# freiberg-roman/mj-grasp-sim

Measured on AMD Instinct MI355X. Metric: grasp candidates evaluated/sec at 200-step horizon, Robotiq2F85xYCB, higher is better.
Workload: dtype f64

## Files before the change

mj-grasp-sim_amd/csrc/mgs_kernels.hip:

```cpp

#include <hip/hip_runtime.h>
#include <stdint.h>

#include "../../include/mgs_gpu.h"

#define K_MINVAL 1e-15
#define K_MAXF 16
#define K_MAXPOLY 40
#define K_POLY_POINTS (4 * K_MAXF + 3 * K_MAXPOLY)
#define K_MPR_MAXIT 64
#define K_FEAT_EPS 1e-5
#define K_BB_MERGE 1e-6
#define K_CERT 8
#define CERT_W 17
#define CERT_STORE 1e-6
#define CERT_EPS 1e-10
#define WAVE 64
#ifndef MGS_GPAD
#ifdef MGS_G_GLOBAL
#define MGS_GPAD 0
#else
#define MGS_GPAD 1
#endif
#endif
// ... 2423 lines not shown
#pragma unroll
  for (int k = 0; k < 3; k++) { a[k] = c.cx1[k]; b[k] = c.cx2[k]; }
}
template <int HW>
DEVI void support_pairq(const PairCtxQ<HW>& c, const double* dir, double* out1, double* out2) {
  const int lane = lane_id(), side = (lane / HW) & 1, li = lane % HW, hb = lane - li;
  double sd[3] = {side ? -dir[0] : dir[0], side ? -dir[1] : dir[1], side ? -dir[2] : dir[2]};
  double dl[3];
  mulmtv3(dl, c.R, sd);
  SupAcc a;
  sup_init(a);
  if (li < c.n) {
    double sc = (c.c[0] * dl[0] + c.c[1] * dl[1]) + c.c[2] * dl[2];
    if (sc > a.best) { a.best = sc; a.bi = li; a.vx = c.c[0]; a.vy = c.c[1]; a.vz = c.c[2]; }
  }
  const int P = c.P;
  double m = a.best;
  if (P > 1) m = max_f64(m, dpp_d(m, 0));
  if (P > 2) m = max_f64(m, dpp_d(m, 1));
  if (P > 4) m = max_f64(m, dpp_d(m, 2));
  if (HW > 8 && P > 8) m = max_f64(m, dpp_d(m, 3));
  const double M = shfl(m, hb);
  const unsigned long long tied = __ballot(a.bi != 0x7fffffff && a.best == M);
  const unsigned tr = (unsigned)(tied >> hb) & ((1u << HW) - 1u);
  const int src = hb + (tr ? __ffs(tr) - 1 : 0);
  double v[3] = {shfl(a.vx, src), shfl(a.vy, src), shfl(a.vz, src)};
  double t[3], wv[3];
  mulmv3(t, c.R, v);
  add3(wv, c.x, t);
  if (c.r > 0.0) { wv[0] = wv[0] + c.r * sd[0]; wv[1] = wv[1] + c.r * sd[1]; wv[2] = wv[2] + c.r * sd[2]; }
  const int s1 = lane - (lane % (2 * HW)), s2 = s1 + HW;
#pragma unroll
  for (int k = 0; k < 3; k++) {
    out1[k] = shfl(wv[k], s1);
    out2[k] = shfl(wv[k], s2);
  }
}
template <int HW>
DEVI void mink_support(const PairCtxQ<HW>& c, const double* dir, SupPt* p, unsigned long long) {
  PT(4);
  PCNT(28, 1);
  support_pairq<HW>(c, dir, p->a, p->b);
  sub3(p->v, p->a, p->b);
  PT(22);
}
#define MQ_P1 0
#define MQ_P2 1
#define MQ_DISC 2
#define MQ_REF 3
#define MQ_PEN 4
#define MQ_FIN 5
#define MQ_DONE 6
template <class QC>
DEVI int ccd_mpr_q(const Mdl& md, const Dat& d, const QC& pc, double* n, double* depth, double* pos) {
  const double tol = md.m.mpr_tolerance;
  const int maxit = md.m.ccd_iterations;
  SupPt p0, p1, p2, p3, ps;
  double dir[3];
  int ph = MQ_P1, it = 0, hit = 0;
  mpr_centres(pc, d, 0, 0, p0.a, p0.b);
  sub3(p0.v, p0.a, p0.b);
  if (ccd_vzero(p0.v)) p0.v[0] = p0.v[0] + CCD_EPS * 10.0;
  dir[0] = -p0.v[0]; dir[1] = -p0.v[1]; dir[2] = -p0.v[2];
  ccd_normalize(dir);
  p1 = p0; p2 = p0; p3 = p0;
  for (;;) {
    if (ph == MQ_REF || ph == MQ_PEN) {
      ccd_portal_dir(dir, p1, p2, p3);
      if (ph == MQ_REF) {
        const double dt = dot3(dir, p1.v);
        if (ccd_iszero(dt) || dt > 0.0) { ph = MQ_PEN; it = 0; }
      }
    }
    const unsigned long long act = __ballot(ph < MQ_FIN);
    if (!act) break;
    mink_support(pc, dir, &ps, act);
    const double dt = dot3(ps.v, dir);
    if (ph == MQ_P1) {
      if (ccd_iszero(dt) || dt < 0.0) {
        ph = MQ_DONE;
      } else {
        p1 = ps;
        cross3(dir, p0.v, p1.v);
        if (ccd_iszero(dot3(dir, dir))) {
          if (!ccd_vzero(p1.v)) {
#pragma unroll
            for (int k = 0; k < 3; k++) { n[k] = p1.v[k]; pos[k] = (p1.a[k] + p1.b[k]) * 0.5; }
            *depth = sqrt(dot3(n, n));
            ccd_normalize(n);
            hit = 1;
          }
          ph = MQ_DONE;
        } else {
          ccd_normalize(dir);
          ph = MQ_P2;
        }
      }
    } else if (ph == MQ_P2) {
      if (ccd_iszero(dt) || dt < 0.0) {
        ph = MQ_DONE;
      } else {
        p2 = ps;
        double e1[3], e2[3];
        sub3(e1, p1.v, p0.v);
        sub3(e2, p2.v, p0.v);
        cross3(dir, e1, e2);
        ccd_normalize(dir);
        if (dot3(dir, p0.v) > 0.0) {
          SupPt tmp = p1; p1 = p2; p2 = tmp;
          dir[0] = -dir[0]; dir[1] = -dir[1]; dir[2] = -dir[2];
        }
        ph = MQ_DISC;
        it = 0;
      }
    } else if (ph == MQ_DISC) {
      if (ccd_iszero(dt) || dt < 0.0) {
        ph = MQ_DONE;
      } else {
        p3 = ps;
        double c[3];
        int cont = 0;
        cross3(c, p1.v, p3.v);
        double dc = dot3(c, p0.v);
        if (dc < 0.0 && !ccd_iszero(dc)) { p2 = p3; cont = 1; }
        if (!cont) {
          cross3(c, p3.v, p2.v);
          dc = dot3(c, p0.v);
          if (dc < 0.0 && !ccd_iszero(dc)) { p1 = p3; cont = 1; }
        }
        if (!cont) {
          ph = MQ_REF;
          it = 0;
        } else {
          double e1[3], e2[3];
          sub3(e1, p1.v, p0.v);
          sub3(e2, p2.v, p0.v);
          cross3(dir, e1, e2);
          ccd_normalize(dir);
          if (++it == CCD_MAXLOOP) ph = MQ_DONE;
        }
      }
    } else if (ph == MQ_REF) {
      if (!(ccd_iszero(dt) || dt > 0.0) || ccd_reach_tol(p1, p2, p3, ps, dir, tol)) {
        ph = MQ_DONE;
      } else {
        PORTAL_EXPAND(p0, p1, p2, p3, ps);
        if (++it == CCD_MAXLOOP) ph = MQ_DONE;
      }
    } else if (ph == MQ_PEN) {
      if (ccd_reach_tol(p1, p2, p3, ps, dir, tol) || it > maxit) {
        ph = MQ_FIN;
      } else {
        PORTAL_EXPAND(p0, p1, p2, p3, ps);
        it++;
      }
    }
  }
  double w[3], fp[3];
  const double dep = sqrt(ccd_tri_dist2(p1.v, p2.v, p3.v, w));
  ccd_normalize(w);
  ccd_find_pos(p0, p1, p2, p3, fp);
  if (ph == MQ_FIN && !ccd_iszero(dep)) {
#pragma unroll
    for (int k = 0; k < 3; k++) { n[k] = w[k]; pos[k] = fp[k]; }
    *depth = dep;
    hit = 1;
  }
  return hit;
}

#define MCCD_N 40
#define MCCD_RES 48
#define MCCD_RES2 96
DEVI void mccd_store(Dat& d, int at, int hit, const double* n, const double* pos, const double* cd, double depth,
                     double cm) {
  double* o = (double*)d.poly + at;
#pragma unroll
  for (int i = 0; i < 3; i++) { o[i] = n[i]; o[3 + i] = pos[i]; o[6 + i] = cd[i]; }
  o[9] = depth;
  o[10] = cm;
  o[11] = hit ? 1.0 : 0.0;
}
DEVI void mccd_take_groups(const Mdl& md, Dat& d, int pair, int g1, int g2, int ngroups, int& nc) {
  const double* cp = (const double*)d.poly;
  const int ncmax = md.m.ncon_max;
#pragma unroll 1
  for (int k = 0; k < ngroups; k++) {
    const double* r = cp + MCCD_RES + 12 * k;
    if (r[11] == 0.0) continue;
    double pk[3] = {r[3], r[4], r[5]};
    if (!mccd_is_new(d, nc, pk, mccd_tol(md, g1, g2))) continue;
    double nk[3] = {r[0], r[1], r[2]};
    const double dk = r[9];
    mccd_list_add(d, nc, pk);
    nc++;
    double u1[3], u2[3];
    make_frame(nk, u1, u2);
    if (lane_id() == 0) add_contact(d, ncmax, pair, g1, g2, pk, nk, u1, u2, -dk);
  }
  wsync();
}
template <int HW>
DEVI void multiccd_q(const Mdl& md, Dat& d, int pair, int g1, int g2, const double* n, const double* pos) {
  constexpr int G = WAVE / (2 * HW);
  mccd_list_init(d, pos);
  int nc = 1;
#pragma unroll 1
  for (int q0 = 0; q0 < 4; q0 += G) {
    {
      double t1[3], t2[3];
      make_frame(n, t1, t2);
      PairCtxQ<HW> pc;
      pair_ctxq<HW>(md, d, g1, g2, t1, t2, pos, q0, pc);
      double nn[3], dd = 0.0, pp[3], dir[3] = {0.0, 0.0, 0.0}, cmx = -1.0;
      const int hit = ccd_mpr_q(md, d, pc, nn, &dd, pp);
      const int lane = lane_id();
      if (lane % (2 * HW) == 0) mccd_store(d, MCCD_RES + 12 * (lane / (2 * HW)), hit, nn, pp, dir, dd, cmx);
      wsync();
    }
    mccd_take_groups(md, d, pair, g1, g2, G, nc);
  }
  wsync();
}

#define MCCD_POSE 16
DEVI void mccd_perturb(const Dat& d, Dat& dw, int g1, int g2, const double* n, const double* pv, int q, int at) {
  const int ax = q >> 1, sg = q & 1;
  double t1[3], t2[3];
  make_frame(n, t1, t2);
  double axis[3] = {ax ? t2[0] : t1[0], ax ? t2[1] : t1[1], ax ? t2[2] : t1[2]};
  double s = sg ? MCCD_S : -MCCD_S;
  double* out = (double*)dw.poly + at;
#pragma unroll 1
  for (int side = 0; side < 2; side++) {
    const int g = side ? g2 : g1;
    double qq[4];
    qq[0] = MCCD_C;
    if (side) { qq[1] = -(axis[0] * s); qq[2] = -(axis[1] * s); qq[3] = -(axis[2] * s); }
    else { qq[1] = axis[0] * s; qq[2] = axis[1] * s; qq[3] = axis[2] * s; }
    double M[9], R[9], xg[3], r[3], t[3], xo[3];
#pragma unroll
    for (int k = 0; k < 9; k++) R[k] = d.geom_xmat[9 * g + k];
#pragma unroll
    for (int k = 0; k < 3; k++) xg[k] = d.geom_xpos[3 * g + k];
    quat2mat(M, qq);
    mulmm3(R, M, R);
    sub3(r, xg, pv);
    mulmv3(t, M, r);
    add3(xo, t, pv);
    if (lane_id() == 0) {
#pragma unroll
      for (int k = 0; k < 9; k++) out[9 * side + k] = R[k];
#pragma unroll
      for (int k = 0; k < 3; k++) out[18 + 3 * side + k] = xo[k];
    }
  }
  wsync();
}

#ifndef MGS_MCCD_W
#define MGS_MCCD_W 1
#endif
#define MCCD_POSEW 128
struct PairCtxW {
  PairCtx base;
  const double* pose;
  double cx1[3], cx2[3];
};
DEVI void mpr_centres(const PairCtxW& c, const Dat&, int, int, double* a, double* b) {
#pragma unroll
  for (int k = 0; k < 3; k++) { a[k] = c.cx1[k]; b[k] = c.cx2[k]; }
}
DEVI void mink_support(const PairCtxW& c, const double* dir, SupPt* p, unsigned long long act) {
  const int grp = lane_id() >> 4;
#pragma unroll 1
  for (int g = 0; g < 4; g++) {
    if (!((act >> (16 * g)) & 1ull)) continue;
    double dg[3] = {readlane_d(dir[0], 16 * g), readlane_d(dir[1], 16 * g), readlane_d(dir[2], 16 * g)};
    PairCtx q = c.base;
    const double* P = c.pose + 24 * g;
#pragma unroll
    for (int k = 0; k < 9; k++) { q.R1[k] = P[k]; q.R2[k] = P[9 + k]; }
#pragma unroll
    for (int k = 0; k < 3; k++) { q.x1[k] = P[18 + k]; q.x2[k] = P[21 + k]; }
    SupPt t;
    mink_support(q, dg, &t);
    if (grp == g) {
#pragma unroll
      for (int k = 0; k < 3; k++) { p->a[k] = t.a[k]; p->b[k] = t.b[k]; }
    }
  }
  sub3(p->v, p->a, p->b);
}
#ifndef MGS_MCCD_G
#define MGS_MCCD_G 1
#endif
#ifndef GS_CH
#define GS_CH 4
#endif
struct PairCtxG {
  int n1, n2;
  int nmax1, nmax2;
  const double *V1, *V2;
  double c1[3], c2[3];
  double r1, r2;
  double cy1[2], cy2[2];
  const double* pose;
  double cx1[3], cx2[3];
};
DEVI void pair_ctxg(const Mdl& md, int g1, int g2, const double* pose, PairCtxG& c) {
  const int li = lane_id() & 15;
  const int32_t *ghull = IA(md, geom_hullid), *hadr = IA(md, hull_vertadr), *hnum = IA(md, hull_vertnum);
  const int h1 = ghull[g1], h2 = ghull[g2];
  c.n1 = hnum[h1];
  c.n2 = hnum[h2];
  c.nmax1 = c.n1;
  c.nmax2 = c.n2;
  c.V1 = DA(md, hull_vert) + 3 * hadr[h1];
  c.V2 = DA(md, hull_vert) + 3 * hadr[h2];
  const int i1 = li < c.n1 ? li : 0, i2 = li < c.n2 ? li : 0;
#pragma unroll
  for (int k = 0; k < 3; k++) { c.c1[k] = c.V1[k * c.n1 + i1]; c.c2[k] = c.V2[k * c.n2 + i2]; }
  c.r1 = DA(md, geom_radius)[g1];
  c.r2 = DA(md, geom_radius)[g2];
  const double* cy = DA(md, geom_cyl);
  c.cy1[0] = cy[2 * g1]; c.cy1[1] = cy[2 * g1 + 1];
  c.cy2[0] = cy[2 * g2]; c.cy2[1] = cy[2 * g2 + 1];
  c.pose = pose;
#pragma unroll
  for (int k = 0; k < 3; k++) { c.cx1[k] = pose[18 + k]; c.cx2[k] = pose[21 + k]; }
}
DEVI void mpr_centres(const PairCtxG& c, const Dat&, int, int, double* a, double* b) {
#pragma unroll
  for (int k = 0; k < 3; k++) { a[k] = c.cx1[k]; b[k] = c.cx2[k]; }
}
DEVI int dpp_i(int x, int ctrl_sel) {
  switch (ctrl_sel) {
    case 0: return __builtin_amdgcn_mov_dpp(x, 0xB1, 0xF, 0xF, false);
    case 1: return __builtin_amdgcn_mov_dpp(x, 0x4E, 0xF, 0xF, false);
    case 2: return __builtin_amdgcn_mov_dpp(x, 0x141, 0xF, 0xF, false);
    default: return __builtin_amdgcn_mov_dpp(x, 0x140, 0xF, 0xF, false);
  }
}
DEVI void sup_group(int n, int nmax, const double* V, const double* cached, const double* dl, double* v) {
  const int lane = lane_id(), li = lane & 15;
  SupAcc a;
  sup_init(a);
  if (nmax <= 16) {
    if (li < n) {
      double sc = (cached[0] * dl[0] + cached[1] * dl[1]) + cached[2] * dl[2];
      if (sc > a.best) { a.best = sc; a.bi = li; a.vx = cached[0]; a.vy = cached[1]; a.vz = cached[2]; }
    }
  } else {
#pragma unroll 1
    for (int base = 0; base < nmax; base += GS_CH * 16) {
      double x[GS_CH], y[GS_CH], z[GS_CH];
#pragma unroll
      for (int u = 0; u < GS_CH; u++) {
        const int i = base + u * 16 + li;
        const int ii = i < n ? i : 0;
        x[u] = V[ii]; y[u] = V[n + ii]; z[u] = V[2 * n + ii];
      }
#pragma unroll
      for (int u = 0; u < GS_CH; u++) {
        const int i = base + u * 16 + li;
        double sc = (x[u] * dl[0] + y[u] * dl[1]) + z[u] * dl[2];
        if (i < n && sc > a.best) { a.best = sc; a.bi = i; a.vx = x[u]; a.vy = y[u]; a.vz = z[u]; }
      }
    }
  }
  double m = a.best;
  m = max_f64(m, dpp_d(m, 0));
  m = max_f64(m, dpp_d(m, 1));
  m = max_f64(m, dpp_d(m, 2));
  m = max_f64(m, dpp_d(m, 3));
  int w = a.best == m ? a.bi : 0x7fffffff, t;
  t = dpp_i(w, 0); w = t < w ? t : w;
  t = dpp_i(w, 1); w = t < w ? t : w;
  t = dpp_i(w, 2); w = t < w ? t : w;
  t = dpp_i(w, 3); w = t < w ? t : w;
  if (w == 0x7fffffff) w = 0;
  const int src = (lane - li) + (w & 15);
  v[0] = shfl(a.vx, src);
  v[1] = shfl(a.vy, src);
  v[2] = shfl(a.vz, src);
}
DEVI void support_pairg(const PairCtxG& c, const double* dir, double* out1, double* out2) {
  const double* P = c.pose;
  double nd[3] = {-dir[0], -dir[1], -dir[2]};
  double R[9], dl[3], v[3], t[3], x[3];
#pragma unroll
  for (int k = 0; k < 9; k++) R[k] = P[k];
  mulmtv3(dl, R, dir);
  sup_group(c.n1, c.nmax1, c.V1, c.c1, dl, v);
  if (c.cy1[0] > 0.0) cyl_support(v, c.cy1, dl);
#pragma unroll
  for (int k = 0; k < 3; k++) x[k] = P[18 + k];
  mulmv3(t, R, v);
  add3(out1, x, t);
  if (c.r1 > 0.0) { out1[0] = out1[0] + c.r1 * dir[0]; out1[1] = out1[1] + c.r1 * dir[1]; out1[2] = out1[2] + c.r1 * dir[2]; }
#pragma unroll
  for (int k = 0; k < 9; k++) R[k] = P[9 + k];
  mulmtv3(dl, R, nd);
  sup_group(c.n2, c.nmax2, c.V2, c.c2, dl, v);
  if (c.cy2[0] > 0.0) cyl_support(v, c.cy2, dl);
#pragma unroll
  for (int k = 0; k < 3; k++) x[k] = P[21 + k];
  mulmv3(t, R, v);
  add3(out2, x, t);
  if (c.r2 > 0.0) { out2[0] = out2[0] + c.r2 * nd[0]; out2[1] = out2[1] + c.r2 * nd[1]; out2[2] = out2[2] + c.r2 * nd[2]; }
}
DEVI void mink_support(const PairCtxG& c, const double* dir, SupPt* p, unsigned long long) {
  PT(4);
  PCNT(28, 1);
  PCNT(29, (c.n1 > WAVE) + (c.n2 > WAVE));
  support_pairg(c, dir, p->a, p->b);
  sub3(p->v, p->a, p->b);
  if (c.n1 > WAVE || c.n2 > WAVE) PT(39); else PT(22);
}
DEVI void multiccd_w(const Mdl& md, Dat& d, int pair, int g1, int g2, const double* n, const double* pos) {
  mccd_list_init(d, pos);
#pragma unroll 1
  for (int q = 0; q < 4; q++) mccd_perturb(d, d, g1, g2, n, pos, q, MCCD_POSEW + 24 * q);
  const int lane = lane_id(), grp = lane >> 4;
  {
#if MGS_MCCD_G
    PairCtxG pc;
    pair_ctxg(md, g1, g2, (const double*)d.poly + MCCD_POSEW + 24 * grp, pc);
#else
    PairCtxW pc;
    pair_ctx(md, d, g1, g2, pc.base);
    pc.pose = (const double*)d.poly + MCCD_POSEW;
    const double* P = pc.pose + 24 * grp;
#pragma unroll
    for (int k = 0; k < 3; k++) { pc.cx1[k] = P[18 + k]; pc.cx2[k] = P[21 + k]; }
#endif
    double nn[3], dd = 0.0, pp[3], dir[3] = {0.0, 0.0, 0.0};
    const int hit = ccd_mpr_q(md, d, pc, nn, &dd, pp);
    if ((lane & 15) == 0) mccd_store(d, MCCD_RES + 12 * grp, hit, nn, pp, dir, dd, -1.0);
    wsync();
  }
  int nc = 1;
  mccd_take_groups(md, d, pair, g1, g2, 4, nc);
}

DEVI void collide_convex_mj(const Mdl& md, Dat& d, int pairA, int pairB, int mccd) {
  const int lane = lane_id();
  const int32_t *p1 = IA(md, pair_geom1), *p2 = IA(md, pair_geom2);
  const int32_t *ghull = IA(md, geom_hullid), *hnum = IA(md, hull_vertnum);
  const double* cy = DA(md, geom_cyl);
  const int ncmax = md.m.ncon_max;
  if (pairB >= 0) {
    const int gA1 = p1[pairA], gA2 = p2[pairA], gB1 = p1[pairB], gB2 = p2[pairB];
    PairCtx2 q;
    pair_ctx2(md, d, gA1, gA2, gB1, gB2, q);
    const int g1 = lane < 32 ? gA1 : gB1, g2 = lane < 32 ? gA2 : gB2;
    double n[3], depth, pos[3], cd[3], cm;
    const int hit = ccd_mpr(md, d, q, g1, g2, n, &depth, pos, cd, &cm);
    if ((lane & 31) == 0) mccd_store(d, MCCD_RES2 + 12 * (lane >> 5), hit, n, pos, cd, depth, cm);
    wsync();
  }
  const int np = pairB >= 0 ? 2 : 1;
  const double* cp = (const double*)d.poly;
#pragma unroll 1
  for (int k = 0; k < np; k++) {
    const int pair = k ? pairB : pairA;
    const int G1 = p1[pair], G2 = p2[pair];
    const bool multi = mccd && md.m.ccd_mode == MGS_CCD_MULTI && IA(md, pair_kind)[pair] == MGS_PAIR_CONVEX;
    int nc = 0;
#pragma unroll 1
    for (int it = 0; it < 5; it++) {
      if (it > 0 || pairB < 0) {
        PairCtx pc;
        if (it > 0) {
          mccd_perturb(d, d, G1, G2, cp + MCCD_N, cp, it - 1, MCCD_POSE);
          const double* pz = cp + MCCD_POSE;
          pair_ctx_pose(md, G1, G2, pz, pz + 18, pz + 9, pz + 21, pc);
        } else {
          pair_ctx(md, d, G1, G2, pc);
        }
        double n[3], depth, pos[3], cd[3], cm;
        const int hit = ccd_mpr(md, d, pc, G1, G2, n, &depth, pos, cd, &cm);
        wsync();
        if (lane == 0) mccd_store(d, MCCD_RES, hit, n, pos, cd, depth, cm);
        wsync();
      }
      const double* r = it == 0 && pairB >= 0 ? cp + MCCD_RES2 + 12 * k : cp + MCCD_RES;
      const int hk = r[11] != 0.0;
      if (it == 0) {
        PT(4);
        cert_update(md, d, pair, G1, G2, hk, r + 6, r[10]);
        PCNT(26, 1);
        PCNT(27, hk);
        if (!hk) break;
        double t1[3], t2[3];
        make_frame(r, t1, t2);
        if (lane == 0) add_contact(d, ncmax, pair, G1, G2, r + 3, r, t1, t2, -r[9]);
        wsync();
        if (!multi) break;
        const int nm1 = hnum[ghull[G1]], nm2 = hnum[ghull[G2]];
        const bool cyl = cy[2 * G1] > 0.0 || cy[2 * G2] > 0.0;
        if (MGS_MCCD_Q && !cyl && nm1 <= 8 && nm2 <= 8) {
          double n0[3] = {r[0], r[1], r[2]}, p0[3] = {r[3], r[4], r[5]};
          multiccd_q<8>(md, d, pair, G1, G2, n0, p0);
          break;
        }
        if (MGS_MCCD_W) {
          double n0[3] = {r[0], r[1], r[2]}, p0[3] = {r[3], r[4], r[5]};
          multiccd_w(md, d, pair, G1, G2, n0, p0);
          break;
        }
        if (lane == 0) {
          double* w = (double*)d.poly;
#pragma unroll
          for (int i = 0; i < 3; i++) { w[i] = r[3 + i]; w[MCCD_N + i] = r[i]; }
        }
        wsync();
        nc = 1;
      } else {
        if (!hk) continue;
        double pk[3] = {r[3], r[4], r[5]};
        if (!mccd_is_new(d, nc, pk, mccd_tol(md, G1, G2))) continue;
        double nk[3] = {r[0], r[1], r[2]};
        const double dk = r[9];
        mccd_list_add(d, nc, pk);
        nc++;
        double u1[3], u2[3];
        make_frame(nk, u1, u2);
        if (lane == 0) add_contact(d, ncmax, pair, G1, G2, pk, nk, u1, u2, -dk);
      }
    }
    wsync();
  }
  PT(41);
}

DEVI double kdist3(const double* a, const double* b) {
  double dx[3];
  sub3(dx, a, b);
  return sqrt(dot3(dx, dx));
}
DEVI int raw_sphere_sphere(const double* p1, const double* z1, double r1, const double* p2, const double* z2,
                           double r2, double margin, double* pos, double* n, double* dist) {
  double dd = (kdist3(p1, p2) - r1) - r2;
  if (dd > margin) return 0;
  sub3(n, p2, p1);
  if (normalize3(n) < K_MINVAL) {
    cross3(n, z1, z2);
    normalize3(n);
  }
  double s = r1 + 0.5 * dd;
#pragma unroll
  for (int k = 0; k < 3; k++) pos[k] = p1[k] + n[k] * s;
  *dist = dd;
// ... 282 lines not shown
  for (int k = 0; k < 3; k++)
#pragma unroll
    for (int i = 0; i < 3; i++) { A1[3 * k + i] = R1[3 * i + k]; A2[3 * k + i] = R2[3 * i + k]; }
  const int qa = q < 6 ? 0 : (q - 6) / 3, qb = q < 6 ? 0 : (q - 6) % 3;
  const double* Rf = q < 3 ? R1 : R2;
  const int kf = q < 3 ? q : (q < 6 ? q - 3 : 0);
  double e1[3], e2[3], L[3], cx[3];
#pragma unroll
  for (int i = 0; i < 3; i++) {
    e1[i] = R1[3 * i + qa];
    e2[i] = R2[3 * i + qb];
  }
  cross3(cx, e1, e2);
#pragma unroll
  for (int i = 0; i < 3; i++) L[i] = q < 6 ? Rf[3 * i + kf] : cx[i];
  double ll = dot3(L, L);
  if (ll < 1e-20) return 0;
  double r1 = (h1[0] * fabs(dot3(A1, L)) + h1[1] * fabs(dot3(A1 + 3, L))) + h1[2] * fabs(dot3(A1 + 6, L));
  double r2 = (h2[0] * fabs(dot3(A2, L)) + h2[1] * fabs(dot3(A2 + 3, L))) + h2[2] * fabs(dot3(A2 + 6, L));
  return fabs(dot3(D, L)) > (r1 + r2) + (margin + 1e-12) * sqrt(ll);
}

DEVI unsigned long long obb_separated_wave(const Dat& d, unsigned long long am, int g1, int g2, const double* D,
                                           const double* h1, const double* h2, double margin) {
  const int lane = lane_id(), grp = lane >> 4, q = lane & 15;
  unsigned long long sep = 0ull;
  while (am) {
    unsigned long long m = am;
    for (int t = 0; t < grp; t++) m &= m - 1ull;
    int b = m ? __ffsll((long long)m) - 1 : 0;
    int G1 = shfl(g1, b), G2 = shfl(g2, b);
    double Db[3], h1b[3], h2b[3];
#pragma unroll
    for (int i = 0; i < 3; i++) {
      Db[i] = shfl(D[i], b);
      h1b[i] = shfl(h1[i], b);
      h2b[i] = shfl(h2[i], b);
    }
    double mb = shfl(margin, b);
    int s = 0;
    if (m && q < 15) s = obb_axis_separated(q, d.geom_xmat + 9 * G1, d.geom_xmat + 9 * G2, Db, h1b, h2b, mb);
    unsigned long long sm = __ballot(s);
#pragma unroll
    for (int k = 0; k < 4; k++) {
      if (!am) break;
      int bk = __ffsll((long long)am) - 1;
      if ((sm >> (16 * k)) & 0x7fffull) sep |= 1ull << bk;
      am &= am - 1ull;
    }
  }
  return sep;
}

DEVI void collision(const Mdl& md, Dat& d, int mccd = 1) {
  int lane = lane_id();
  const int32_t *p1 = IA(md, pair_geom1), *p2 = IA(md, pair_geom2);
  const double *aabb = DA(md, geom_aabb), *pm = DA(md, pair_margin);
  if (lane == 0) d.NCON = 0;
  wsync();
  int npair = md.m.npair;
  for (int c0 = 0; c0 < npair; c0 += WAVE) {
    int p = c0 + lane;
    int ov = 0;
    int g[2] = {0, 0};
    double c[2][3], hw[2][3], D[3] = {0.0, 0.0, 0.0}, h[2][3] = {{0.0, 0.0, 0.0}, {0.0, 0.0, 0.0}}, mp = 0.0;
    if (p < npair) {
      g[0] = p1[p];
      g[1] = p2[p];
      mp = pm[p];
      for (int s = 0; s < 2; s++) {
        const double* R = d.geom_xmat + 9 * g[s];
        const double* lc = aabb + 6 * g[s];
        const double* lh = lc + 3;
        double t[3];
        mulmv3(t, R, lc);
        add3(c[s], d.geom_xpos + 3 * g[s], t);
        for (int k = 0; k < 3; k++) {
          h[s][k] = lh[k];
          hw[s][k] = (fabs(R[3 * k]) * lh[0] + fabs(R[3 * k + 1]) * lh[1]) + fabs(R[3 * k + 2]) * lh[2];
        }
      }
      ov = 1;
      for (int k = 0; k < 3; k++)
        if (fabs(c[0][k] - c[1][k]) > (hw[0][k] + hw[1][k]) + mp) ov = 0;
      sub3(D, c[1], c[0]);
    }
    PT(59);
    int small2 = 0;
    const int pk = p < npair ? IA(md, pair_kind)[p] : MGS_PAIR_BOXBOX;
    const bool mpr_pair = md.m.ccd_mode == MGS_CCD_R5 ? pk != MGS_PAIR_BOXBOX
                                                       : (pk == MGS_PAIR_CONVEX || pk == MGS_PAIR_CONVEX_SMOOTH);
    if (ov && mpr_pair) {
      const int32_t *ghull = IA(md, geom_hullid), *hnum = IA(md, hull_vertnum);
      small2 = hnum[ghull[g[0]]] <= 16 && hnum[ghull[g[1]]] <= 16;
    }
    const unsigned long long smallm = __ballot(small2);
    unsigned long long mask = __ballot(ov);
    mask &= ~obb_separated_wave(d, mask, g[0], g[1], D, h[0], h[1], mp);
    PT(60);
    mask &= ~cert_check(md, d, c0, mask);
    PT(3);
    while (mask) {
      int b = __ffsll((long long)mask) - 1;
      mask &= mask - 1ull;
      const int kind = IA(md, pair_kind)[c0 + b];
      if (((smallm >> b) & 1ull) && mask && ((smallm >> (__ffsll((long long)mask) - 1)) & 1ull)) {
        int b2 = __ffsll((long long)mask) - 1;
        mask &= mask - 1ull;
        if (md.m.ccd_mode == MGS_CCD_R5) collide_pair2(md, d, c0 + b, c0 + b2);
        else collide_convex_mj(md, d, c0 + b, c0 + b2, mccd);
      } else if (kind == MGS_PAIR_BOXBOX) {
        collide_boxbox(md, d, c0 + b);
      } else if (md.m.ccd_mode == MGS_CCD_R5) {
        collide_pair(md, d, c0 + b);
      } else if (kind == MGS_PAIR_CONVEX || kind == MGS_PAIR_CONVEX_SMOOTH) {
        collide_convex_mj(md, d, c0 + b, -1, mccd);
      } else {
        collide_prim(md, d, c0 + b, kind);
      }
    }
  }
}

enum {
  L_qpos, L_qvel, L_qacc_ws, L_ctrl, L_mocap_pos, L_mocap_quat, L_time, L_act, L_act_dot,
  L_xpos, L_xquat, L_xmat, L_subtree_com, L_cinert, L_cdof,
  L_M, L_Dv, L_Dinv, L_sD, L_isD, L_tmp, L_tmp2,
  L_qfrc_smooth, L_qacc_smooth, L_qfrc_constraint,
  L_act_force, L_act_moment, L_act_length, L_act_vel,
  L_con_pos, L_con_frame, L_con_dist, L_con_mu, L_con_blk,
  L_efc_R, L_efc_b, L_cert,
  L_U, L_ints, L_COUNT
};
enum {
  U_poly, U_pdep, U_geom_xpos, U_geom_xmat, U_xipos, U_xanchor, U_xaxis, U_subtree_mass, U_comacc,
  U_crb, U_cvel, U_cacc, U_cfrc, U_cdof_dot, U_qfrc_bias, U_qfrc_passive, U_qfrc_actuator,
  U_G, U_aref, U_vel, U_pos, U_margin, U_nH, U_scratch, U_jar, U_jv, U_f, U_Dr, U_isR, U_nw, U_nw0, U_ng,
  U_ndir, U_qDeriv, U_COUNT
};
#ifndef MGS_HBM_EXTRA
#define MGS_HBM_EXTRA 0
#endif
DEVI size_t hbm_slice(int ne, int nv, int nc) {
  return (size_t)ne * nv + (MGS_HBM_EXTRA ? (size_t)(K_CERT * CERT_W + 9 * nc + BLKSTRIDE * nc) : 0);
}
struct Lay {
  int o[L_COUNT];
  int u[U_COUNT];
  int ncon_max, nefc_max, nv;
  int total_doubles;
  double* gmem;
};

#ifdef MGS_SPECIAL
#include MGS_SPECIAL
static_assert(MGS_SL_ABI == MGS_ABI_VERSION, "specialisation header of another ABI version: regenerate it");
static_assert(MGS_SL_DESC_BYTES == sizeof(mgs_model_desc), "specialisation header of another mgs_model_desc");
#else
#define MGS_SL_NV 0
constexpr int mgs_sl_words[L_COUNT + U_COUNT + 4] = {0};
constexpr mgs_model_desc mgs_sl_desc = {};
#endif
static_assert(sizeof(mgs_sl_words) == sizeof(int) * (L_COUNT + U_COUNT + 4), "specialised layout size");

template <int SL>
DEVI void bind(Dat& d, double* s, const Lay& l) {
#define LO(k) (SL ? mgs_sl_words[k] : l.o[k])
#define LU(k) (SL ? mgs_sl_words[L_COUNT + (k)] : l.u[k])
#define B(f) d.f = s + LO(L_##f)
  B(qpos); B(qvel); B(qacc_ws); B(ctrl); B(mocap_pos); B(mocap_quat); B(time); B(act); B(act_dot);
  B(xpos); B(xquat); B(xmat); B(subtree_com); B(cinert); B(cdof);
// ... 2761 lines not shown
```

Measured before the change: 391,900.

## Batch first MPR of up to four convex pairs across 16-lane groups

Adds collide_chunk_mj, which runs the initial MPR for up to four overlapping convex pairs at once, one pair per 16-lane group, then processes each pair's contact, cert update and multi-CCD perturbation from the stored results. Previously pairs were handled one or two at a time with the whole wave busy on each. ccd_mpr_q now also returns the last direction and a separation certificate value, and skips the final portal distance work when no lane finished in penetration. Per-group radius and cylinder data move from registers into shared scratch. The cost is more scratch-layout coupling and extra wave syncs, and some groups sit idle when fewer than four convex pairs are available.

```diff
diff --git a/mj-grasp-sim_amd/csrc/mgs_kernels.hip b/mj-grasp-sim_amd/csrc/mgs_kernels.hip
--- a/mj-grasp-sim_amd/csrc/mgs_kernels.hip
+++ b/mj-grasp-sim_amd/csrc/mgs_kernels.hip
@@ -2499,12 +2499,13 @@
 #define MQ_FIN 5
 #define MQ_DONE 6
 template <class QC>
-DEVI int ccd_mpr_q(const Mdl& md, const Dat& d, const QC& pc, double* n, double* depth, double* pos) {
+DEVI int ccd_mpr_q(const Mdl& md, const Dat& d, const QC& pc, double* n, double* depth, double* pos, double* cd,
+                   double* cm, int live = 1) {
   const double tol = md.m.mpr_tolerance;
   const int maxit = md.m.ccd_iterations;
   SupPt p0, p1, p2, p3, ps;
-  double dir[3];
-  int ph = MQ_P1, it = 0, hit = 0;
+  double dir[3], cert = -1.0;
+  int ph = live ? MQ_P1 : MQ_DONE, it = 0, hit = 0;
   mpr_centres(pc, d, 0, 0, p0.a, p0.b);
   sub3(p0.v, p0.a, p0.b);
   if (ccd_vzero(p0.v)) p0.v[0] = p0.v[0] + CCD_EPS * 10.0;
@@ -2525,6 +2526,7 @@
     const double dt = dot3(ps.v, dir);
     if (ph == MQ_P1) {
       if (ccd_iszero(dt) || dt < 0.0) {
+        cert = -dt;
         ph = MQ_DONE;
       } else {
         p1 = ps;
@@ -2545,6 +2547,7 @@
       }
     } else if (ph == MQ_P2) {
       if (ccd_iszero(dt) || dt < 0.0) {
+        cert = -dt;
         ph = MQ_DONE;
       } else {
         p2 = ps;
@@ -2562,6 +2565,7 @@
       }
     } else if (ph == MQ_DISC) {
       if (ccd_iszero(dt) || dt < 0.0) {
+        cert = -dt;
         ph = MQ_DONE;
       } else {
         p3 = ps;
@@ -2588,7 +2592,10 @@
         }
       }
     } else if (ph == MQ_REF) {
-      if (!(ccd_iszero(dt) || dt > 0.0) || ccd_reach_tol(p1, p2, p3, ps, dir, tol)) {
+      if (!(ccd_iszero(dt) || dt > 0.0)) {
+        cert = -dt;
+        ph = MQ_DONE;
+      } else if (ccd_reach_tol(p1, p2, p3, ps, dir, tol)) {
         ph = MQ_DONE;
       } else {
         PORTAL_EXPAND(p0, p1, p2, p3, ps);
@@ -2603,16 +2610,20 @@
       }
     }
   }
-  double w[3], fp[3];
-  const double dep = sqrt(ccd_tri_dist2(p1.v, p2.v, p3.v, w));
-  ccd_normalize(w);
-  ccd_find_pos(p0, p1, p2, p3, fp);
-  if (ph == MQ_FIN && !ccd_iszero(dep)) {
-#pragma unroll
-    for (int k = 0; k < 3; k++) { n[k] = w[k]; pos[k] = fp[k]; }
-    *depth = dep;
-    hit = 1;
-  }
+  if (__ballot(ph == MQ_FIN)) {
+    double w[3], fp[3];
+    const double dep = sqrt(ccd_tri_dist2(p1.v, p2.v, p3.v, w));
+    ccd_normalize(w);
+    ccd_find_pos(p0, p1, p2, p3, fp);
+    if (ph == MQ_FIN && !ccd_iszero(dep)) {
+#pragma unroll
+      for (int k = 0; k < 3; k++) { n[k] = w[k]; pos[k] = fp[k]; }
+      *depth = dep;
+      hit = 1;
+    }
+  }
+  cd[0] = dir[0]; cd[1] = dir[1]; cd[2] = dir[2];
+  *cm = cert;
   return hit;
 }
 
@@ -2660,7 +2671,7 @@
       PairCtxQ<HW> pc;
       pair_ctxq<HW>(md, d, g1, g2, t1, t2, pos, q0, pc);
       double nn[3], dd = 0.0, pp[3], dir[3] = {0.0, 0.0, 0.0}, cmx = -1.0;
-      const int hit = ccd_mpr_q(md, d, pc, nn, &dd, pp);
+      const int hit = ccd_mpr_q(md, d, pc, nn, &dd, pp, dir, &cmx);
       const int lane = lane_id();
       if (lane % (2 * HW) == 0) mccd_store(d, MCCD_RES + 12 * (lane / (2 * HW)), hit, nn, pp, dir, dd, cmx);
       wsync();
@@ -2709,6 +2720,7 @@
 #define MGS_MCCD_W 1
 #endif
 #define MCCD_POSEW 128
+#define MCCD_GEO 224
 struct PairCtxW {
   PairCtx base;
   const double* pose;
@@ -2750,12 +2762,11 @@
   int nmax1, nmax2;
   const double *V1, *V2;
   double c1[3], c2[3];
-  double r1, r2;
-  double cy1[2], cy2[2];
+  const double* geo;
   const double* pose;
   double cx1[3], cx2[3];
 };
-DEVI void pair_ctxg(const Mdl& md, int g1, int g2, const double* pose, PairCtxG& c) {
+DEVI void pair_ctxg(const Mdl& md, int g1, int g2, const double* pose, double* geo, PairCtxG& c) {
   const int li = lane_id() & 15;
   const int32_t *ghull = IA(md, geom_hullid), *hadr = IA(md, hull_vertadr), *hnum = IA(md, hull_vertnum);
   const int h1 = ghull[g1], h2 = ghull[g2];
@@ -2768,11 +2779,12 @@
   const int i1 = li < c.n1 ? li : 0, i2 = li < c.n2 ? li : 0;
 #pragma unroll
   for (int k = 0; k < 3; k++) { c.c1[k] = c.V1[k * c.n1 + i1]; c.c2[k] = c.V2[k * c.n2 + i2]; }
-  c.r1 = DA(md, geom_radius)[g1];
-  c.r2 = DA(md, geom_radius)[g2];
-  const double* cy = DA(md, geom_cyl);
-  c.cy1[0] = cy[2 * g1]; c.cy1[1] = cy[2 * g1 + 1];
-  c.cy2[0] = cy[2 * g2]; c.cy2[1] = cy[2 * g2 + 1];
+  if (li < 6) {
+    const int g = (li == 0 || li == 2 || li == 3) ? g1 : g2;
+    geo[li] = li < 2 ? DA(md, geom_radius)[g] : DA(md, geom_cyl)[2 * g + (li & 1)];
+  }
+  wsync();
+  c.geo = geo;
   c.pose = pose;
 #pragma unroll
   for (int k = 0; k < 3; k++) { c.cx1[k] = pose[18 + k]; c.cx2[k] = pose[21 + k]; }
@@ -2840,22 +2852,23 @@
   for (int k = 0; k < 9; k++) R[k] = P[k];
   mulmtv3(dl, R, dir);
   sup_group(c.n1, c.nmax1, c.V1, c.c1, dl, v);
-  if (c.cy1[0] > 0.0) cyl_support(v, c.cy1, dl);
+  if (c.geo[2] > 0.0) cyl_support(v, c.geo + 2, dl);
 #pragma unroll
   for (int k = 0; k < 3; k++) x[k] = P[18 + k];
   mulmv3(t, R, v);
   add3(out1, x, t);
-  if (c.r1 > 0.0) { out1[0] = out1[0] + c.r1 * dir[0]; out1[1] = out1[1] + c.r1 * dir[1]; out1[2] = out1[2] + c.r1 * dir[2]; }
+  const double r1 = c.geo[0], r2 = c.geo[1];
+  if (r1 > 0.0) { out1[0] = out1[0] + r1 * dir[0]; out1[1] = out1[1] + r1 * dir[1]; out1[2] = out1[2] + r1 * dir[2]; }
 #pragma unroll
   for (int k = 0; k < 9; k++) R[k] = P[9 + k];
   mulmtv3(dl, R, nd);
   sup_group(c.n2, c.nmax2, c.V2, c.c2, dl, v);
-  if (c.cy2[0] > 0.0) cyl_support(v, c.cy2, dl);
+  if (c.geo[4] > 0.0) cyl_support(v, c.geo + 4, dl);
 #pragma unroll
   for (int k = 0; k < 3; k++) x[k] = P[21 + k];
   mulmv3(t, R, v);
   add3(out2, x, t);
-  if (c.r2 > 0.0) { out2[0] = out2[0] + c.r2 * nd[0]; out2[1] = out2[1] + c.r2 * nd[1]; out2[2] = out2[2] + c.r2 * nd[2]; }
+  if (r2 > 0.0) { out2[0] = out2[0] + r2 * nd[0]; out2[1] = out2[1] + r2 * nd[1]; out2[2] = out2[2] + r2 * nd[2]; }
 }
 DEVI void mink_support(const PairCtxG& c, const double* dir, SupPt* p, unsigned long long) {
   PT(4);
@@ -2873,7 +2886,7 @@
   {
 #if MGS_MCCD_G
     PairCtxG pc;
-    pair_ctxg(md, g1, g2, (const double*)d.poly + MCCD_POSEW + 24 * grp, pc);
+    pair_ctxg(md, g1, g2, (const double*)d.poly + MCCD_POSEW + 24 * grp, (double*)d.poly + MCCD_GEO + 6 * grp, pc);
 #else
     PairCtxW pc;
     pair_ctx(md, d, g1, g2, pc.base);
@@ -2882,9 +2895,9 @@
 #pragma unroll
     for (int k = 0; k < 3; k++) { pc.cx1[k] = P[18 + k]; pc.cx2[k] = P[21 + k]; }
 #endif
-    double nn[3], dd = 0.0, pp[3], dir[3] = {0.0, 0.0, 0.0};
-    const int hit = ccd_mpr_q(md, d, pc, nn, &dd, pp);
-    if ((lane & 15) == 0) mccd_store(d, MCCD_RES + 12 * grp, hit, nn, pp, dir, dd, -1.0);
+    double nn[3], dd = 0.0, pp[3], dir[3], cmx;
+    const int hit = ccd_mpr_q(md, d, pc, nn, &dd, pp, dir, &cmx);
+    if ((lane & 15) == 0) mccd_store(d, MCCD_RES + 12 * grp, hit, nn, pp, dir, dd, cmx);
     wsync();
   }
   int nc = 1;
@@ -3335,6 +3348,129 @@
   return sep;
 }
 
+#ifndef MGS_MPR1_G
+#ifdef MGS_WAVES_PER_EU
+#define MGS_MPR1_G 0
+#else
+#define MGS_MPR1_G 1
+#endif
+#endif
+#if MGS_MPR1_G && !(MGS_MCCD_W && MGS_MCCD_G)
+#error "MGS_MPR1_G 1 shares multiccd_w's group-scan MPR call site: it needs MGS_MCCD_W 1 and MGS_MCCD_G 1"
+#endif
+#define MPR1_POSE (K_POLY_POINTS * 3 - 4 * 24)
+#define MPR1_RES (MPR1_POSE - 4 * 12)
+static_assert(MPR1_POSE + 4 * 24 == K_POLY_POINTS * 3, "the first-MPR block ends with the polygon scratch");
+static_assert(MPR1_RES >= MCCD_GEO + 4 * 6 && MCCD_GEO >= MCCD_POSEW + 4 * 24 && MPR1_RES >= MCCD_RES + 4 * 12 &&
+                  MCCD_GEO >= 3 * 48,
+              "the first-MPR block overlaps multiccd's or collide_boxbox's scratch");
+#if MGS_MPR1_G
+DEVI void collide_chunk_mj(const Mdl& md, Dat& d, int c0, unsigned long long mask, unsigned long long cvx, int mccd) {
+  const int lane = lane_id(), grp = lane >> 4, li = lane & 15;
+  const int32_t *p1 = IA(md, pair_geom1), *p2 = IA(md, pair_geom2);
+  const int32_t *ghull = IA(md, geom_hullid), *hnum = IA(md, hull_vertnum);
+  const double* cy = DA(md, geom_cyl);
+  const int ncmax = md.m.ncon_max;
+  double* cp = (double*)d.poly;
+  unsigned long long batch = 0ull;
+  while (mask) {
+    const int b = __ffsll((long long)mask) - 1;
+    const int pair = c0 + b;
+    if (!((cvx >> b) & 1ull)) {
+      const int kind = IA(md, pair_kind)[pair];
+      if (kind == MGS_PAIR_BOXBOX) collide_boxbox(md, d, pair);
+      else collide_prim(md, d, pair, kind);
+      mask &= mask - 1ull;
+      continue;
+    }
+    const int G1 = p1[pair], G2 = p2[pair];
+    const bool multi = mccd && md.m.ccd_mode == MGS_CCD_MULTI && IA(md, pair_kind)[pair] == MGS_PAIR_CONVEX;
+#pragma unroll 1
+    for (int st = 0; st < 2; st++) {
+      int ga = G1, gb = G2, live = 1, at = MCCD_RES + 12 * grp, posat = MCCD_POSEW + 24 * grp;
+      if (st == 0) {
+        if ((batch >> b) & 1ull) continue;
+        unsigned long long m = mask & cvx;
+        int bg = -1;
+        batch = 0ull;
+#pragma unroll
+        for (int k = 0; k < 4; k++) {
+          if (!m) break;
+          const int bk = __ffsll((long long)m) - 1;
+          m &= m - 1ull;
+          batch |= 1ull << bk;
+          if (grp == k) bg = bk;
+        }
+        live = bg >= 0;
+        if (!live) bg = b;
+        ga = p1[c0 + bg];
+        gb = p2[c0 + bg];
+        at = MPR1_RES + 12 * grp;
+        posat = MPR1_POSE + 24 * grp;
+#pragma unroll
+        for (int u = 0; u < 2; u++) {
+          const int v = li + 16 * u;
+          if (v < 24) {
+            double x;
+            if (v < 9) x = d.geom_xmat[9 * ga + v];
+            else if (v < 18) x = d.geom_xmat[9 * gb + (v - 9)];
+            else if (v < 21) x = d.geom_xpos[3 * ga + (v - 18)];
+            else x = d.geom_xpos[3 * gb + (v - 21)];
+            cp[posat + v] = x;
+          }
+        }
+        wsync();
+      } else {
+        const double* r = cp + MPR1_RES + 12 * __popcll(batch & ((1ull << b) - 1ull));
+        const int hk = r[11] != 0.0;
+        PT(4);
+        cert_update(md, d, pair, G1, G2, hk, r + 6, r[10]);
+        PCNT(26, 1);
+        PCNT(27, hk);
+        if (!hk) continue;
+        double t1[3], t2[3];
+        make_frame(r, t1, t2);
+        if (lane == 0) add_contact(d, ncmax, pair, G1, G2, r + 3, r, t1, t2, -r[9]);
+        wsync();
+        if (!multi) continue;
+        const int nm1 = hnum[ghull[G1]], nm2 = hnum[ghull[G2]];
+        const bool cyl = cy[2 * G1] > 0.0 || cy[2 * G2] > 0.0;
+        double n0[3] = {r[0], r[1], r[2]}, p0[3] = {r[3], r[4], r[5]};
+        if (MGS_MCCD_Q && !cyl && nm1 <= 8 && nm2 <= 8) {
+          multiccd_q<8>(md, d, pair, G1, G2, n0, p0);
+          continue;
+        }
+        mccd_list_init(d, p0);
+#pragma unroll 1
+        for (int q = 0; q < 4; q++) mccd_perturb(d, d, G1, G2, n0, p0, q, MCCD_POSEW + 24 * q);
+      }
+      {
+        PairCtxG pc;
+        pair_ctxg(md, ga, gb, cp + posat, cp + MCCD_GEO + 6 * grp, pc);
+#pragma unroll
+        for (int k = 1; k < 4; k++) {
+          const int a1 = __builtin_amdgcn_readlane(pc.n1, 16 * k), a2 = __builtin_amdgcn_readlane(pc.n2, 16 * k);
+          pc.nmax1 = a1 > pc.nmax1 ? a1 : pc.nmax1;
+          pc.nmax2 = a2 > pc.nmax2 ? a2 : pc.nmax2;
+        }
+        pc.nmax1 = __builtin_amdgcn_readfirstlane(pc.nmax1);
+        pc.nmax2 = __builtin_amdgcn_readfirstlane(pc.nmax2);
+        double nn[3], dd = 0.0, pp[3], cd[3], cm;
+        const int hit = ccd_mpr_q(md, d, pc, nn, &dd, pp, cd, &cm, live);
+        if (li == 0 && live) mccd_store(d, at, hit, nn, pp, cd, dd, cm);
+        wsync();
+      }
+      if (st == 1) {
+        int nc = 1;
+        mccd_take_groups(md, d, pair, G1, G2, 4, nc);
+      }
+    }
+    PT(41);
+    mask &= mask - 1ull;
+  }
+}
+#endif
+
 DEVI void collision(const Mdl& md, Dat& d, int mccd = 1) {
   int lane = lane_id();
   const int32_t *p1 = IA(md, pair_geom1), *p2 = IA(md, pair_geom2);
@@ -3373,7 +3509,7 @@
     const int pk = p < npair ? IA(md, pair_kind)[p] : MGS_PAIR_BOXBOX;
     const bool mpr_pair = md.m.ccd_mode == MGS_CCD_R5 ? pk != MGS_PAIR_BOXBOX
                                                        : (pk == MGS_PAIR_CONVEX || pk == MGS_PAIR_CONVEX_SMOOTH);
-    if (ov && mpr_pair) {
+    if (ov && mpr_pair && (!MGS_MPR1_G || md.m.ccd_mode == MGS_CCD_R5)) {
       const int32_t *ghull = IA(md, geom_hullid), *hnum = IA(md, hull_vertnum);
       small2 = hnum[ghull[g[0]]] <= 16 && hnum[ghull[g[1]]] <= 16;
     }
@@ -3383,6 +3519,12 @@
     PT(60);
     mask &= ~cert_check(md, d, c0, mask);
     PT(3);
+#if MGS_MPR1_G
+    if (md.m.ccd_mode != MGS_CCD_R5) {
+      collide_chunk_mj(md, d, c0, mask, __ballot(mpr_pair), mccd);
+      continue;
+    }
+#endif
     while (mask) {
       int b = __ffsll((long long)mask) - 1;
       mask &= mask - 1ull;
@@ -3391,15 +3533,19 @@
         int b2 = __ffsll((long long)mask) - 1;
         mask &= mask - 1ull;
         if (md.m.ccd_mode == MGS_CCD_R5) collide_pair2(md, d, c0 + b, c0 + b2);
+#if !MGS_MPR1_G
         else collide_convex_mj(md, d, c0 + b, c0 + b2, mccd);
+#endif
       } else if (kind == MGS_PAIR_BOXBOX) {
         collide_boxbox(md, d, c0 + b);
       } else if (md.m.ccd_mode == MGS_CCD_R5) {
         collide_pair(md, d, c0 + b);
+#if !MGS_MPR1_G
       } else if (kind == MGS_PAIR_CONVEX || kind == MGS_PAIR_CONVEX_SMOOTH) {
         collide_convex_mj(md, d, c0 + b, -1, mccd);
       } else {
         collide_prim(md, d, c0 + b, kind);
+#endif
       }
     }
   }
```

Result: no change. 391,600, median of 3 (-0.1%).

## Batch multi-CCD perturbation MPR across up to four convex pairs per wave

Applied to the files above, without the earlier changes.

Adds a cross-pair batching path for multi-CCD. Eligible small convex pairs (at most 8 hull vertices, not cylinders) first run their base MPR and store it to scratch, then all their perturbed MPRs run together in one wave at 16 lanes per pair and 4 lanes per perturbation. Contacts are emitted from the batched results afterwards. This targets the serial per-pair multiccd_q calls that underuse the wave, at the cost of more complex scheduling, extra scratch use and dummy lanes when fewer than two pairs are live.

```diff
diff --git a/mj-grasp-sim_amd/csrc/mgs_kernels.hip b/mj-grasp-sim_amd/csrc/mgs_kernels.hip
--- a/mj-grasp-sim_amd/csrc/mgs_kernels.hip
+++ b/mj-grasp-sim_amd/csrc/mgs_kernels.hip
@@ -2499,12 +2499,12 @@
 #define MQ_FIN 5
 #define MQ_DONE 6
 template <class QC>
-DEVI int ccd_mpr_q(const Mdl& md, const Dat& d, const QC& pc, double* n, double* depth, double* pos) {
+DEVI int ccd_mpr_q(const Mdl& md, const Dat& d, const QC& pc, double* n, double* depth, double* pos, int done0 = 0) {
   const double tol = md.m.mpr_tolerance;
   const int maxit = md.m.ccd_iterations;
   SupPt p0, p1, p2, p3, ps;
   double dir[3];
-  int ph = MQ_P1, it = 0, hit = 0;
+  int ph = done0 ? MQ_DONE : MQ_P1, it = 0, hit = 0;
   mpr_centres(pc, d, 0, 0, p0.a, p0.b);
   sub3(p0.v, p0.a, p0.b);
   if (ccd_vzero(p0.v)) p0.v[0] = p0.v[0] + CCD_EPS * 10.0;
@@ -2619,6 +2619,9 @@
 #define MCCD_N 40
 #define MCCD_RES 48
 #define MCCD_RES2 96
+#define MCCD_XRES1 224
+#define MCCD_XRES 272
+static_assert(MCCD_XRES + 16 * 12 <= K_POLY_POINTS * 3, "multiccd_x results past the polygon scratch");
 DEVI void mccd_store(Dat& d, int at, int hit, const double* n, const double* pos, const double* cd, double depth,
                      double cm) {
   double* o = (double*)d.poly + at;
@@ -2628,12 +2631,13 @@
   o[10] = cm;
   o[11] = hit ? 1.0 : 0.0;
 }
-DEVI void mccd_take_groups(const Mdl& md, Dat& d, int pair, int g1, int g2, int ngroups, int& nc) {
+DEVI void mccd_take_groups(const Mdl& md, Dat& d, int pair, int g1, int g2, int ngroups, int& nc,
+                           int at = MCCD_RES) {
   const double* cp = (const double*)d.poly;
   const int ncmax = md.m.ncon_max;
 #pragma unroll 1
   for (int k = 0; k < ngroups; k++) {
-    const double* r = cp + MCCD_RES + 12 * k;
+    const double* r = cp + at + 12 * k;
     if (r[11] == 0.0) continue;
     double pk[3] = {r[3], r[4], r[5]};
     if (!mccd_is_new(d, nc, pk, mccd_tol(md, g1, g2))) continue;
@@ -2891,7 +2895,163 @@
   mccd_take_groups(md, d, pair, g1, g2, 4, nc);
 }
 
-DEVI void collide_convex_mj(const Mdl& md, Dat& d, int pairA, int pairB, int mccd) {
+#ifndef MGS_MCCD_X
+#define MGS_MCCD_X 1
+#endif
+#ifndef MGS_MCCD_XV
+#define MGS_MCCD_XV 1
+#endif
+struct PairCtxX {
+  int n1, n2;
+  double R1[9], R2[9], x1[3], x2[3];
+#if MGS_MCCD_XV
+  double v1[2][3], v2[2][3];
+#else
+  const double *v1, *v2;
+#endif
+  double r1, r2;
+};
+DEVI void xpose(const Dat& d, int g, const double* qq, const double* pv, double* R, double* x) {
+  double M[9], Rg[9], xg[3], r[3], t[3];
+  quat2mat(M, qq);
+#pragma unroll
+  for (int k = 0; k < 9; k++) Rg[k] = d.geom_xmat[9 * g + k];
+#pragma unroll
+  for (int k = 0; k < 3; k++) xg[k] = d.geom_xpos[3 * g + k];
+  mulmm3(R, M, Rg);
+  sub3(r, xg, pv);
+  mulmv3(t, M, r);
+  add3(x, t, pv);
+}
+DEVI void pair_ctxx(const Mdl& md, const Dat& d, int pair, const double* n0, const double* pv, int q, PairCtxX& c) {
+  const int li = lane_id() & 3;
+  const int g1 = IA(md, pair_geom1)[pair], g2 = IA(md, pair_geom2)[pair];
+  const int32_t *ghull = IA(md, geom_hullid), *hadr = IA(md, hull_vertadr), *hnum = IA(md, hull_vertnum);
+  const int h1 = ghull[g1], h2 = ghull[g2];
+  c.n1 = hnum[h1];
+  c.n2 = hnum[h2];
+  const double* V1 = DA(md, hull_vert) + 3 * hadr[h1];
+  const double* V2 = DA(md, hull_vert) + 3 * hadr[h2];
+#if MGS_MCCD_XV
+#pragma unroll
+  for (int u = 0; u < 2; u++) {
+    const int i = li + 4 * u;
+    const int i1 = i < c.n1 ? i : 0, i2 = i < c.n2 ? i : 0;
+#pragma unroll
+    for (int k = 0; k < 3; k++) { c.v1[u][k] = V1[k * c.n1 + i1]; c.v2[u][k] = V2[k * c.n2 + i2]; }
+  }
+#else
+  c.v1 = V1;
+  c.v2 = V2;
+#endif
+  c.r1 = DA(md, geom_radius)[g1];
+  c.r2 = DA(md, geom_radius)[g2];
+  const int ax = q >> 1, sg = q & 1;
+  double t1[3], t2[3];
+  make_frame(n0, t1, t2);
+  double axis[3] = {ax ? t2[0] : t1[0], ax ? t2[1] : t1[1], ax ? t2[2] : t1[2]};
+  double s = sg ? MCCD_S : -MCCD_S;
+  double qa[4] = {MCCD_C, axis[0] * s, axis[1] * s, axis[2] * s};
+  double qb[4] = {MCCD_C, -(axis[0] * s), -(axis[1] * s), -(axis[2] * s)};
+  xpose(d, g1, qa, pv, c.R1, c.x1);
+  xpose(d, g2, qb, pv, c.R2, c.x2);
+}
+DEVI void mpr_centres(const PairCtxX& c, const Dat&, int, int, double* a, double* b) {
+#pragma unroll
+  for (int k = 0; k < 3; k++) { a[k] = c.x1[k]; b[k] = c.x2[k]; }
+}
+#if MGS_MCCD_XV
+DEVI void sup_quad(int n, const double (*V)[3], const double* dl, double* v) {
+  const int lane = lane_id(), li = lane & 3;
+#else
+DEVI void sup_quad(int n, const double* Vg, const double* dl, double* v) {
+  const int lane = lane_id(), li = lane & 3;
+  double V[2][3];
+#pragma unroll
+  for (int u = 0; u < 2; u++) {
+    const int i = li + 4 * u < n ? li + 4 * u : 0;
+#pragma unroll
+    for (int k = 0; k < 3; k++) V[u][k] = Vg[k * n + i];
+  }
+#endif
+  SupAcc a;
+  sup_init(a);
+#pragma unroll
+  for (int u = 0; u < 2; u++) {
+    const int i = li + 4 * u;
+    double sc = (V[u][0] * dl[0] + V[u][1] * dl[1]) + V[u][2] * dl[2];
+    if (i < n && sc > a.best) { a.best = sc; a.bi = i; a.vx = V[u][0]; a.vy = V[u][1]; a.vz = V[u][2]; }
+  }
+  double m = a.best;
+  m = max_f64(m, dpp_d(m, 0));
+  m = max_f64(m, dpp_d(m, 1));
+  int w = a.best == m ? a.bi : 0x7fffffff, t;
+  t = dpp_i(w, 0); w = t < w ? t : w;
+  t = dpp_i(w, 1); w = t < w ? t : w;
+  if (w == 0x7fffffff) w = 0;
+  const int src = (lane - li) + (w & 3);
+  v[0] = shfl(a.vx, src);
+  v[1] = shfl(a.vy, src);
+  v[2] = shfl(a.vz, src);
+}
+DEVI void support_pairx(const PairCtxX& c, const double* dir, double* out1, double* out2) {
+  double nd[3] = {-dir[0], -dir[1], -dir[2]};
+  double dl[3], v[3], t[3];
+  mulmtv3(dl, c.R1, dir);
+  sup_quad(c.n1, c.v1, dl, v);
+  mulmv3(t, c.R1, v);
+  add3(out1, c.x1, t);
+  if (c.r1 > 0.0) { out1[0] = out1[0] + c.r1 * dir[0]; out1[1] = out1[1] + c.r1 * dir[1]; out1[2] = out1[2] + c.r1 * dir[2]; }
+  mulmtv3(dl, c.R2, nd);
+  sup_quad(c.n2, c.v2, dl, v);
+  mulmv3(t, c.R2, v);
+  add3(out2, c.x2, t);
+  if (c.r2 > 0.0) { out2[0] = out2[0] + c.r2 * nd[0]; out2[1] = out2[1] + c.r2 * nd[1]; out2[2] = out2[2] + c.r2 * nd[2]; }
+}
+DEVI void mink_support(const PairCtxX& c, const double* dir, SupPt* p, unsigned long long) {
+  PT(4);
+  PCNT(28, 1);
+  support_pairx(c, dir, p->a, p->b);
+  sub3(p->v, p->a, p->b);
+  PT(22);
+}
+DEVI int multiccd_x(const Mdl& md, Dat& d, int c0, unsigned long long xall) {
+  const int lane = lane_id(), slot = lane >> 4;
+  const double* cp = (const double*)d.poly;
+  int pair = -1;
+  {
+    unsigned long long t = xall;
+#pragma unroll
+    for (int s = 0; s < 4; s++) {
+      if (!t) break;
+      const int b = __ffsll((long long)t) - 1;
+      t &= t - 1ull;
+      if (slot == s) pair = c0 + b;
+    }
+  }
+  const int live = pair >= 0 && cp[MCCD_XRES1 + 12 * slot + 11] != 0.0;
+  const unsigned long long lm = __ballot(live);
+  if (__popcll(lm) < 2 * 16) return 0;
+  const int fl = __ffsll((long long)lm) - 1;
+  const int ps = live ? pair : __builtin_amdgcn_readlane(pair, fl);
+  const double* r = cp + MCCD_XRES1 + 12 * (live ? slot : fl >> 4);
+  {
+    double n0[3] = {r[0], r[1], r[2]}, pv[3] = {r[3], r[4], r[5]};
+    PairCtxX pc;
+    pair_ctxx(md, d, ps, n0, pv, (lane >> 2) & 3, pc);
+    double nn[3] = {0.0, 0.0, 0.0}, dd = 0.0, pp[3] = {0.0, 0.0, 0.0}, dir[3] = {0.0, 0.0, 0.0};
+    const int hit = ccd_mpr_q(md, d, pc, nn, &dd, pp, !live);
+    if ((lane & 3) == 0) mccd_store(d, MCCD_XRES + 12 * (lane >> 2), hit, nn, pp, dir, dd, -1.0);
+    wsync();
+  }
+  return 1;
+}
+
+#define CX_ALL 0
+#define CX_FIRST 1
+#define CX_EMIT 2
+DEVI void collide_convex_mj(const Mdl& md, Dat& d, int pairA, int pairB, int mccd, int xmode = CX_ALL,
+                            int xslot = 0, int xran = 0) {
   const int lane = lane_id();
   const int32_t *p1 = IA(md, pair_geom1), *p2 = IA(md, pair_geom2);
   const int32_t *ghull = IA(md, geom_hullid), *hnum = IA(md, hull_vertnum);
@@ -2904,8 +3064,10 @@
     const int g1 = lane < 32 ? gA1 : gB1, g2 = lane < 32 ? gA2 : gB2;
     double n[3], depth, pos[3], cd[3], cm;
     const int hit = ccd_mpr(md, d, q, g1, g2, n, &depth, pos, cd, &cm);
-    if ((lane & 31) == 0) mccd_store(d, MCCD_RES2 + 12 * (lane >> 5), hit, n, pos, cd, depth, cm);
+    const int at = xmode == CX_FIRST ? MCCD_XRES1 + 12 * xslot : MCCD_RES2;
+    if ((lane & 31) == 0) mccd_store(d, at + 12 * (lane >> 5), hit, n, pos, cd, depth, cm);
     wsync();
+    if (xmode == CX_FIRST) return;
   }
   const int np = pairB >= 0 ? 2 : 1;
   const double* cp = (const double*)d.poly;
@@ -2917,7 +3079,7 @@
     int nc = 0;
 #pragma unroll 1
     for (int it = 0; it < 5; it++) {
-      if (it > 0 || pairB < 0) {
+      if (it > 0 || (pairB < 0 && xmode != CX_EMIT)) {
         PairCtx pc;
         if (it > 0) {
           mccd_perturb(d, d, G1, G2, cp + MCCD_N, cp, it - 1, MCCD_POSE);
@@ -2929,10 +3091,13 @@
         double n[3], depth, pos[3], cd[3], cm;
         const int hit = ccd_mpr(md, d, pc, G1, G2, n, &depth, pos, cd, &cm);
         wsync();
-        if (lane == 0) mccd_store(d, MCCD_RES, hit, n, pos, cd, depth, cm);
+        if (lane == 0) mccd_store(d, xmode == CX_FIRST ? MCCD_XRES1 + 12 * xslot : MCCD_RES, hit, n, pos, cd, depth, cm);
         wsync();
-      }
-      const double* r = it == 0 && pairB >= 0 ? cp + MCCD_RES2 + 12 * k : cp + MCCD_RES;
+        if (xmode == CX_FIRST) break;
+      }
+      const double* r = it == 0 && xmode == CX_EMIT ? cp + MCCD_XRES1 + 12 * xslot
+                        : it == 0 && pairB >= 0     ? cp + MCCD_RES2 + 12 * k
+                                                    : cp + MCCD_RES;
       const int hk = r[11] != 0.0;
       if (it == 0) {
         PT(4);
@@ -2947,6 +3112,13 @@
         if (!multi) break;
         const int nm1 = hnum[ghull[G1]], nm2 = hnum[ghull[G2]];
         const bool cyl = cy[2 * G1] > 0.0 || cy[2 * G2] > 0.0;
+        if (xmode == CX_EMIT && xran) {
+          double p0[3] = {r[3], r[4], r[5]};
+          mccd_list_init(d, p0);
+          nc = 1;
+          mccd_take_groups(md, d, pair, G1, G2, 4, nc, MCCD_XRES + 48 * xslot);
+          break;
+        }
         if (MGS_MCCD_Q && !cyl && nm1 <= 8 && nm2 <= 8) {
           double n0[3] = {r[0], r[1], r[2]}, p0[3] = {r[3], r[4], r[5]};
           multiccd_q<8>(md, d, pair, G1, G2, n0, p0);
@@ -3369,35 +3541,62 @@
       sub3(D, c[1], c[0]);
     }
     PT(59);
-    int small2 = 0;
+    int small2 = 0, xel = 0;
     const int pk = p < npair ? IA(md, pair_kind)[p] : MGS_PAIR_BOXBOX;
     const bool mpr_pair = md.m.ccd_mode == MGS_CCD_R5 ? pk != MGS_PAIR_BOXBOX
                                                        : (pk == MGS_PAIR_CONVEX || pk == MGS_PAIR_CONVEX_SMOOTH);
     if (ov && mpr_pair) {
       const int32_t *ghull = IA(md, geom_hullid), *hnum = IA(md, hull_vertnum);
-      small2 = hnum[ghull[g[0]]] <= 16 && hnum[ghull[g[1]]] <= 16;
+      const int n1 = hnum[ghull[g[0]]], n2 = hnum[ghull[g[1]]];
+      small2 = n1 <= 16 && n2 <= 16;
+      const double* cy = DA(md, geom_cyl);
+      xel = MGS_MCCD_X && MGS_MCCD_Q && mccd && md.m.ccd_mode == MGS_CCD_MULTI && pk == MGS_PAIR_CONVEX &&
+            n1 <= 8 && n2 <= 8 && !(cy[2 * g[0]] > 0.0 || cy[2 * g[1]] > 0.0);
     }
     const unsigned long long smallm = __ballot(small2);
+    unsigned long long xelm = __ballot(xel);
     unsigned long long mask = __ballot(ov);
     mask &= ~obb_separated_wave(d, mask, g[0], g[1], D, h[0], h[1], mp);
     PT(60);
     mask &= ~cert_check(md, d, c0, mask);
     PT(3);
+    unsigned long long xall = 0ull, xq = 0ull;
+    int xran = 0;
     while (mask) {
-      int b = __ffsll((long long)mask) - 1;
-      mask &= mask - 1ull;
+      int b = __ffsll((long long)mask) - 1, b2 = -1, xmode = CX_ALL, xslot = 0;
+      if (xq) {
+        b = __ffsll((long long)xq) - 1;
+        xq &= xq - 1ull;
+        if (xq) { b2 = __ffsll((long long)xq) - 1; xq &= xq - 1ull; }
+        xmode = CX_FIRST;
+      } else if (((xelm & ~xall) >> b) & 1ull) {
+        unsigned long long t = xelm & mask;
+        xall = 0ull;
+        for (int s = 0; s < 4 && t; s++) { xall |= t & (0ull - t); t &= t - 1ull; }
+        if (xall & (xall - 1ull)) { xq = xall; continue; }
+        xelm &= ~xall;
+        xall = 0ull;
+      }
+      if (xmode != CX_FIRST) {
+        mask &= mask - 1ull;
+        if ((xall >> b) & 1ull) {
+          xmode = CX_EMIT;
+        } else if (((smallm >> b) & 1ull) && mask && ((smallm & ~xall) >> (__ffsll((long long)mask) - 1)) & 1ull) {
+          b2 = __ffsll((long long)mask) - 1;
+          mask &= mask - 1ull;
+        }
+      }
+      if (xmode != CX_ALL) xslot = __popcll(xall & ((1ull << b) - 1ull));
       const int kind = IA(md, pair_kind)[c0 + b];
-      if (((smallm >> b) & 1ull) && mask && ((smallm >> (__ffsll((long long)mask) - 1)) & 1ull)) {
-        int b2 = __ffsll((long long)mask) - 1;
-        mask &= mask - 1ull;
-        if (md.m.ccd_mode == MGS_CCD_R5) collide_pair2(md, d, c0 + b, c0 + b2);
-        else collide_convex_mj(md, d, c0 + b, c0 + b2, mccd);
+      if (md.m.ccd_mode == MGS_CCD_R5 && b2 >= 0) {
+        collide_pair2(md, d, c0 + b, c0 + b2);
       } else if (kind == MGS_PAIR_BOXBOX) {
         collide_boxbox(md, d, c0 + b);
       } else if (md.m.ccd_mode == MGS_CCD_R5) {
         collide_pair(md, d, c0 + b);
       } else if (kind == MGS_PAIR_CONVEX || kind == MGS_PAIR_CONVEX_SMOOTH) {
-        collide_convex_mj(md, d, c0 + b, -1, mccd);
+        collide_convex_mj(md, d, c0 + b, b2 >= 0 ? c0 + b2 : -1, mccd, xmode, xslot, xran);
+        if (xmode == CX_FIRST && !xq) xran = multiccd_x(md, d, c0, xall);
       } else {
         collide_prim(md, d, c0 + b, kind);
       }
```

Result: faster. 392,200 before, 410,500 after (median of 6 runs) (+4.7%).
